# lenskit/lkpy

Hardware: AMD Instinct MI355X
Metric: ALS-implicit epochs/sec (ML-25M-shaped, k=64) (higher is better)
Workload: dtype f32; 1 GPU; MovieLens-25M-shaped, als-implicit k=64, 829 timed epochs, 1 x MI355X; solver=cholesky, n_items=62423, nnz=25000095, parallelism=single GPU

## Files before the change

### include/lkamd.h

```cpp
#ifndef LKAMD_H
#define LKAMD_H

#include <stddef.h>
#include <stdint.h>

#ifdef __cplusplus
extern "C" {
#endif

#define LK_OK 0
#define LK_E_INVALID (-1)
#define LK_E_HIP (-2)
#define LK_E_NOT_SPD (-3)
#define LK_E_NAN_SIM (-4)
#define LK_E_NOMEM (-5)
#define LK_E_CANCELLED (-6)

#define LK_SOLVER_CHOLESKY 0
#define LK_SOLVER_CG 1
#define LK_SOLVER_AUTO 2

const char *lk_last_error(void);
const char *lk_version(void);
int lk_device_count(void);
// ... 7 lines not shown

typedef struct lk_task_ctl lk_task_ctl;
int lk_task_ctl_create(lk_task_ctl **out);
void lk_task_ctl_destroy(lk_task_ctl *ctl);
void lk_task_ctl_cancel(lk_task_ctl *ctl);
int lk_task_ctl_cancelled(const lk_task_ctl *ctl);
void lk_task_ctl_reset(lk_task_ctl *ctl);
int lk_task_ctl_progress(const lk_task_ctl *ctl, int64_t *rows_done, int64_t *rows_total);

size_t lk_gramian_workspace_bytes(int32_t k);
int lk_gramian(const float *d_m, int64_t n, int32_t k, int32_t ld, float reg, float *d_out,
               int32_t ld_out, void *d_ws, void *stream);

typedef struct lk_als_plan lk_als_plan;

int lk_als_plan_create(lk_als_plan **out, const void *h_indptr, int indptr_is_64, int64_t n_rows,
                       int32_t k, int32_t solver);
#define LK_ALS_PLAN_REFERENCE_ORDER 1
#define LK_ALS_PLAN_HYBRID_ORDER 2
int lk_als_plan_create_ex(lk_als_plan **out, const void *h_indptr, int indptr_is_64,
                          int64_t n_rows, int32_t k, int32_t solver, int32_t flags);
void lk_als_plan_destroy(lk_als_plan *plan);
int64_t lk_als_plan_long_rows(const lk_als_plan *plan);
const float *lk_als_plan_yref(const lk_als_plan *plan, const void *d_ws);
size_t lk_als_plan_workspace_bytes(const lk_als_plan *plan);
int32_t lk_als_plan_solver(const lk_als_plan *plan);

int lk_als_plan_set_cg(lk_als_plan *plan, float tol, int32_t max_iter);
int lk_als_plan_cg_stats(const lk_als_plan *plan, void *d_ws, void *stream,
                         int64_t *out_iterations, int64_t *out_rows);
int lk_als_plan_set_ctl(lk_als_plan *plan, lk_task_ctl *ctl);
int64_t lk_als_plan_short_rows(const lk_als_plan *plan);
int64_t lk_als_plan_woodbury_rows(const lk_als_plan *plan);
int lk_als_plan_set_z(lk_als_plan *plan, const float *d_z);
int lk_als_plan_set_z_workspace(lk_als_plan *plan, float *d_zbuf);
int lk_als_plan_set_rhs_workspace(lk_als_plan *plan, float *d_y);
int lk_als_plan_set_z_shared(lk_als_plan *plan, const float *d_z, const void *d_flag);
int lk_als_plan_set_z_leader(lk_als_plan *plan, int on);
const void *lk_als_plan_z_flag(const lk_als_plan *plan, const void *d_ws);
size_t lk_spd_inverse_workspace_bytes(int32_t k);
int lk_spd_inverse(const float *d_a, int32_t lda, int32_t k, float *d_out, int32_t *d_flag,
                   void *d_ws, void *stream);

int lk_als_implicit_half_epoch(const lk_als_plan *plan, const void *d_indptr,
                               const int32_t *d_indices, const float *d_values, int64_t n_rows,
                               int64_t n_cols, int32_t k, float *d_this, int32_t ld_this,
// ... 410 lines not shown
```

### lkpy_amd/_native.py

```python

from __future__ import annotations

import ctypes
import os
import re
from ctypes import POINTER, c_char_p, c_float, c_int, c_int32, c_int64, c_size_t, c_void_p
from pathlib import Path

_PKG = Path(__file__).resolve().parent
LIB_PATH = Path(os.environ.get("LK_AMD_LIBRARY", _PKG / "_lkamd.so"))
HEADER_PATH = _PKG.parent / "include" / "lkamd.h"

LK_OK = 0
LK_E_INVALID = -1
LK_E_HIP = -2
LK_E_NOT_SPD = -3
LK_E_NAN_SIM = -4
LK_E_NOMEM = -5
LK_E_CANCELLED = -6

SOLVER_CHOLESKY = 0
SOLVER_CG = 1
SOLVER_AUTO = 2

# ... 49 lines not shown
        "lk_task_ctl_create": (c_int, [POINTER(vp)]),
        "lk_task_ctl_destroy": (None, [vp]),
        "lk_task_ctl_cancel": (None, [vp]),
        "lk_task_ctl_cancelled": (c_int, [vp]),
        "lk_task_ctl_reset": (None, [vp]),
        "lk_task_ctl_progress": (c_int, [vp, POINTER(c_int64), POINTER(c_int64)]),
        "lk_als_plan_set_ctl": (c_int, [vp, vp]),
        "lk_iknn_plan_set_ctl": (c_int, [vp, vp]),
        "lk_iknn_plan_enable_timing": (c_int, [vp, c_int]),
        "lk_iknn_plan_get_timing": (c_int, [vp, POINTER(ctypes.c_double), POINTER(c_int32)]),
        "lk_argtopn_workspace_bytes": (c_size_t, [c_int64, c_int64, c_int32]),
        "lk_gramian_workspace_bytes": (c_size_t, [c_int32]),
        "lk_gramian": (c_int, [vp, c_int64, c_int32, c_int32, c_float, vp, c_int32, vp, vp]),
        "lk_als_plan_create": (c_int, [POINTER(vp), vp, c_int, c_int64, c_int32, c_int32]),
        "lk_als_plan_create_ex": (c_int, [POINTER(vp), vp, c_int, c_int64, c_int32, c_int32,
                                          c_int32]),
        "lk_als_plan_destroy": (None, [vp]),
        "lk_als_plan_workspace_bytes": (c_size_t, [vp]),
        "lk_als_plan_solver": (c_int32, [vp]),
        "lk_als_plan_set_cg": (c_int, [vp, c_float, c_int32]),
        "lk_als_plan_cg_stats": (c_int, [vp, vp, vp, POINTER(c_int64), POINTER(c_int64)]),
        "lk_als_plan_short_rows": (c_int64, [vp]),
        "lk_als_plan_long_rows": (c_int64, [vp]),
        "lk_als_plan_yref": (vp, [vp, vp]),
        "lk_als_plan_woodbury_rows": (c_int64, [vp]),
        "lk_als_plan_set_z": (c_int, [vp, vp]),
        "lk_als_plan_set_z_workspace": (c_int, [vp, vp]),
        "lk_als_plan_set_rhs_workspace": (c_int, [vp, vp]),
        "lk_als_plan_set_z_shared": (c_int, [vp, vp, vp]),
        "lk_als_plan_set_z_leader": (c_int, [vp, c_int]),
        "lk_als_plan_z_flag": (vp, [vp, vp]),
        "lk_spd_inverse_workspace_bytes": (c_size_t, [c_int32]),
        "lk_spd_inverse": (c_int, [vp, c_int32, c_int32, vp, vp, vp, vp]),
        "lk_als_implicit_half_epoch": (
            c_int,
            [vp, vp, vp, vp, c_int64, c_int64, c_int32, vp, c_int32, vp, c_int32, vp, c_int32, vp,
             vp, vp],
        ),
        "lk_als_implicit_epoch": (
            c_int,
            [vp, vp, vp, vp, vp, vp, vp, vp, c_int32, vp, vp, vp, c_int32, c_float, vp, c_int32,
             c_float, vp, vp, vp, vp, vp],
        ),
        "lk_als_explicit_half_epoch": (
            c_int,
            [vp, vp, vp, vp, c_int64, c_int64, c_int32, vp, c_int32, vp, c_int32, c_float, vp, vp,
# ... 307 lines not shown
```

### lkpy_amd/csrc/als_chol.hip

```cpp
#include <algorithm>
#include <utility>

#include "als_plan.h"
#include "common.h"
#include "delta_reduce.h"

#ifndef LK_ALS_RING
#define LK_ALS_RING 4
#endif

namespace lk {

#ifdef LK_ALS_PHASES
__device__ unsigned *lk_als_phase_buf;
#define LK_PHASE_T(var) const unsigned long long var = __builtin_amdgcn_s_memtime()
#define LK_PHASE_ADD(i, a, b) \
    if (lane_id() == 0 && lk_als_phase_buf) lk_als_phase_buf[t * 8 + (i)] = (unsigned)((b) - (a))
#else
#define LK_PHASE_T(var)
#define LK_PHASE_ADD(i, a, b)
#endif

__host__ __device__ constexpr int als_tiles(int NT) { return NT * (NT + 1) / 2; }
__host__ __device__ constexpr int tidx(int ti, int tj) { return tj * (tj + 1) / 2 + ti; }
// ... 48 lines not shown
        q[3] = t.w;
    }
}

template <int NT>
struct GatherRing {
    static constexpr int RING = LK_ALS_RING;
    float q[RING][NT];
    float v[RING];
};

template <int NT>
__device__ __forceinline__ void ring_issue(GatherRing<NT> &R, const int slot_idx, const int g,
                                           const float *stage_slot,
                                           const float *__restrict__ other)
{
    constexpr int KP = NT * 16;
    const int lane = lane_id();
    const int col = __builtin_bit_cast(int, stage_slot[g * 4]);
    R.v[slot_idx] = stage_slot[64 + g * 4];
    load_q<NT>(other + (int64_t)col * KP + (lane & 15) * NT, R.q[slot_idx]);
}

template <int NT, bool MASKED, bool SEQY = false>
__device__ __forceinline__ void ring_consume(Gram<NT> &G, const GatherRing<NT> &R,
                                             const int slot_idx, const int g, const int nb,
                                             const bool expl)
{
    const int lane = lane_id();
    const bool live = !MASKED || (g * 4 + (lane >> 4)) < nb;
    const float v = R.v[slot_idx];
    const float va = expl ? 1.0f : v;
    float q[NT], a[NT];
#pragma unroll
    for (int t = 0; t < NT; ++t) {
        q[t] = live ? R.q[slot_idx][t] : 0.f;
        a[t] = q[t] * va;
    }
#pragma unroll
    for (int tj = 0; tj < NT; ++tj)
#pragma unroll
        for (int ti = 0; ti <= tj; ++ti)
            G.t[tidx(ti, tj)] = __builtin_amdgcn_mfma_f32_16x16x4f32(a[ti], q[tj],
                                                                     G.t[tidx(ti, tj)], 0, 0, 0);
    const float v1 = expl ? v : v + 1.0f;
    if constexpr (SEQY) {
        y_chain_step<NT>(G.yc, q, v1);
    } else {
#pragma unroll
        for (int t = 0; t < NT; ++t) G.y[t] = fmaf(q[t], v1, G.y[t]);
    }
}

constexpr int GRAM_STAGE_WORDS = 256;

template <int NT, bool SEQY = false>
__device__ __forceinline__ void gram_accumulate(Gram<NT> &G, const int32_t *__restrict__ cols,
                                                const float *__restrict__ vals, int64_t beg,
                                                int64_t end, const float *__restrict__ other,
                                                int , const bool expl,
                                                float *stage )
{
    const int lane = lane_id();
    constexpr int RING = GatherRing<NT>::RING;
    static_assert(RING >= 1 && RING <= 8 && 16 % RING == 0, "gather ring: 1, 2, 4 or 8 slots");
    GatherRing<NT> R;
    const int64_t last = end - 1;

    float *wr_cur = stage + lane, *wr_nxt = stage + 128 + lane;
    const float *rd_cur = stage + (lane >> 4), *rd_nxt = stage + 128 + (lane >> 4);
    int nxt_col;
    float nxt_val;
    {
        const int64_t e = (beg + lane < end) ? beg + lane : last;
        wr_cur[0] = __builtin_bit_cast(float, cols[e]);
        wr_cur[64] = vals[e];
    }
#pragma unroll
    for (int g = 0; g < RING; ++g) ring_issue<NT>(R, g, g, rd_cur, other);

    int64_t base = beg;
    for (; base + 64 <= end; base += 64) {
        {
            const int64_t e = (base + 64 + lane < end) ? base + 64 + lane : last;
            nxt_col = cols[e];
            nxt_val = vals[e];
        }
#pragma unroll
        for (int g = 0; g < 16; ++g) {
            ring_consume<NT, false, SEQY>(G, R, g % RING, g, 64, expl);
            if (g == 16 - RING - 2) {
                wr_nxt[0] = __builtin_bit_cast(float, nxt_col);
                wr_nxt[64] = nxt_val;
            }
            if (g < 16 - RING)
                ring_issue<NT>(R, g % RING, g + RING, rd_cur, other);
            else
                ring_issue<NT>(R, g % RING, g + RING - 16, rd_nxt, other);
            __builtin_amdgcn_sched_barrier(0);
        }
        float *tw = wr_cur;
        wr_cur = wr_nxt;
        wr_nxt = tw;
        const float *tr = rd_cur;
        rd_cur = rd_nxt;
        rd_nxt = tr;
    }
    if (base < end) {
        const int nb = (int)(end - base);
        const int ngroups = (nb + 3) >> 2;
#pragma unroll
        for (int g = 0; g < 16; ++g) {
            if (g < ngroups) ring_consume<NT, true, SEQY>(G, R, g % RING, g, nb, expl);
            if (g < 16 - RING) ring_issue<NT>(R, g % RING, g + RING, rd_cur, other);
        }
    }
}

#ifndef LK_ALS_DMA_RING
#define LK_ALS_DMA_RING 8
#endif
constexpr int DMA_RING = LK_ALS_DMA_RING;
constexpr int GRAM_DMA_WORDS = DMA_RING * 256;

template <int N>
__device__ __forceinline__ void wait_vm()
{
    asm volatile("s_waitcnt vmcnt(%0)" ::"n"(N) : "memory");
}
__device__ __forceinline__ void wait_vm_upto(const int n)
{
    if (n >= 7) wait_vm<7>();
    else if (n == 6) wait_vm<6>();
    else if (n == 5) wait_vm<5>();
    else if (n == 4) wait_vm<4>();
    else if (n == 3) wait_vm<3>();
    else if (n == 2) wait_vm<2>();
    else if (n == 1) wait_vm<1>();
    else wait_vm<0>();
}

__device__ __forceinline__ void dma_issue(const unsigned ring_lds, const int slot_idx, const int g,
                                          const float *stage_slot,
                                          const float *__restrict__ other)
{
    const int lane = lane_id();
// ... 3 lines not shown
    const unsigned dst = ring_lds + slot_idx * 1024;
    unsigned keep;
    asm volatile(
        "s_mov_b32 %0, m0\n\ts_mov_b32 m0, %2\n\ts_nop 0\n\t"
        "global_load_lds_dwordx4 %1, off\n\ts_mov_b32 m0, %0"
        : "=&s"(keep)
        : "v"(src), "s"(dst)
        : "memory");
}

struct DmaOperand {
    f32x4 q;
    float v;
};
__device__ __forceinline__ DmaOperand dma_fetch(const float *ring, const int slot_idx, const int g,
                                                const float *stage_slot)
{
    DmaOperand o;
    o.q = *reinterpret_cast<const f32x4 *>(ring + slot_idx * 256 + lane_id() * 4);
    o.v = stage_slot[64 + g * 4];
    return o;
}

template <bool MASKED, bool SEQY = false>
__device__ __forceinline__ void dma_apply(Gram<4> &G, const DmaOperand &o, const int g,
                                          const int nb, const bool expl)
{
    const int lane = lane_id();
    const bool live = !MASKED || (g * 4 + (lane >> 4)) < nb;
    const float v = o.v;
    const float va = expl ? 1.0f : v;
    float q[4] = {o.q.x, o.q.y, o.q.z, o.q.w}, a[4];
#pragma unroll
    for (int t = 0; t < 4; ++t) {
        q[t] = live ? q[t] : 0.f;
        a[t] = q[t] * va;
    }
#pragma unroll
    for (int tj = 0; tj < 4; ++tj)
#pragma unroll
        for (int ti = 0; ti <= tj; ++ti)
            G.t[tidx(ti, tj)] = __builtin_amdgcn_mfma_f32_16x16x4f32(a[ti], q[tj],
                                                                     G.t[tidx(ti, tj)], 0, 0, 0);
    const float v1 = expl ? v : v + 1.0f;
    if constexpr (SEQY) {
        y_chain_step<4>(G.yc, q, v1);
    } else {
#pragma unroll
        for (int t = 0; t < 4; ++t) G.y[t] = fmaf(q[t], v1, G.y[t]);
    }
}

template <bool MASKED, bool SEQY = false>
__device__ __forceinline__ void dma_consume(Gram<4> &G, const float *ring, const int slot_idx,
                                            const int g, const int nb, const float *stage_slot,
                                            const bool expl)
{
    dma_apply<MASKED, SEQY>(G, dma_fetch(ring, slot_idx, g, stage_slot), g, nb, expl);
}

template <int NT>
__host__ __device__ constexpr int slab_floats();
template <int NT>
__device__ __forceinline__ void slab_store(const Gram<NT> &G, float *__restrict__ slab);
template <int NT>
__device__ __forceinline__ void gram_zero(Gram<NT> &G);

template <bool SEQY = false>
__device__ __forceinline__ void gram_accumulate_dma(Gram<4> &G, const int32_t *__restrict__ cols,
                                                    const float *__restrict__ vals, int64_t beg,
                                                    int64_t end, const float *__restrict__ other,
                                                    const bool expl, float *ring, float *stage,
                                                    float *__restrict__ slab = nullptr)
{
    constexpr int RING = DMA_RING;
    static_assert(RING == 8 || RING == 4, "DMA ring: 4 or 8 groups");
    const int lane = lane_id();
    const int64_t last = end - 1;
    const unsigned ring_lds =
        __builtin_amdgcn_readfirstlane((unsigned)(uintptr_t) reinterpret_cast<void *>(ring));

    float *wr_cur = stage + lane, *wr_nxt = stage + 128 + lane;
    const float *rd_cur = stage + (lane >> 4), *rd_nxt = stage + 128 + (lane >> 4);
    {
        const int64_t e = (beg + lane < end) ? beg + lane : last;
        wr_cur[0] = __builtin_bit_cast(float, cols[e]);
        wr_cur[64] = vals[e];
    }
    const int total = (int)((end - beg + 3) >> 2);
#pragma unroll
    for (int g = 0; g < RING; ++g)
        if (g < total) dma_issue(ring_lds, g, g, rd_cur, other);

    int64_t base = beg;
    int g0 = 0;
    for (; g0 + 16 + RING <= total; base += 64, g0 += 16) {
        int nxt_col;
        float nxt_val;
        {
            const int64_t e = (base + 64 + lane < end) ? base + 64 + lane : last;
            nxt_col = cols[e];
            nxt_val = vals[e];
        }
        wait_vm<RING - 1>();
        DmaOperand cur = dma_fetch(ring, 0, 0, rd_cur);
#pragma unroll
        for (int g = 0; g < 16; ++g) {
            DmaOperand nxt = cur;
            if (g + 1 < 16) {
                wait_vm<RING - 2>();
                nxt = dma_fetch(ring, (g + 1) % RING, g + 1, rd_cur);
            }
            dma_apply<false, SEQY>(G, cur, g, 64, expl);
            if (g == 16 - RING - 2) {
                wr_nxt[0] = __builtin_bit_cast(float, nxt_col);
                wr_nxt[64] = nxt_val;
            }
            if (g < 16 - RING)
                dma_issue(ring_lds, g % RING, g + RING, rd_cur, other);
            else
                dma_issue(ring_lds, g % RING, g + RING - 16, rd_nxt, other);
            cur = nxt;
            __builtin_amdgcn_sched_barrier(0);
        }
        if (slab && ((g0 + 16) & 63) == 0) {
            slab_store<4>(G, slab);
            slab += slab_floats<4>();
            gram_zero<4>(G);
        }
        float *tw = wr_cur;
        wr_cur = wr_nxt;
        wr_nxt = tw;
        const float *tr = rd_cur;
        rd_cur = rd_nxt;
        rd_nxt = tr;
    }
    for (; g0 < total; base += 64, g0 += 16) {
        const int nb = (int)((end - base < 64) ? end - base : 64);
        const bool more = g0 + 16 < total;
        int nxt_col = 0;
        float nxt_val = 0.f;
        if (more) {
            const int64_t e = (base + 64 + lane < end) ? base + 64 + lane : last;
            nxt_col = cols[e];
            nxt_val = vals[e];
        }
#pragma unroll
        for (int g = 0; g < 16; ++g) {
            const int gg = g0 + g;
            if (gg < total) {
                const int later = total - 1 - gg;
                wait_vm_upto(later < RING - 1 ? later : RING - 1);
                dma_consume<true, SEQY>(G, ring, g % RING, g, nb, rd_cur, expl);
            }
            if (g == 16 - RING - 2 && more) {
                wr_nxt[0] = __builtin_bit_cast(float, nxt_col);
                wr_nxt[64] = nxt_val;
            }
            if (gg + RING < total) {
                if (g < 16 - RING)
                    dma_issue(ring_lds, g % RING, g + RING, rd_cur, other);
                else
                    dma_issue(ring_lds, g % RING, g + RING - 16, rd_nxt, other);
            }
        }
        if (slab && ((g0 + 16) & 63) == 0 && g0 + 16 < total) {
            slab_store<4>(G, slab);
            slab += slab_floats<4>();
            gram_zero<4>(G);
        }
        float *tw = wr_cur;
        wr_cur = wr_nxt;
        wr_nxt = tw;
        const float *tr = rd_cur;
        rd_cur = rd_nxt;
        rd_nxt = tr;
    }
}

__device__ __forceinline__ void gram_accumulate_dma_256(Gram<4> &G, const int32_t *__restrict__ cols,
                                                        const float *__restrict__ vals, int64_t beg,
                                                        const float *__restrict__ other,
                                                        const bool expl, float *ring, float *stage)
{
    constexpr int RING = DMA_RING, TOTAL = 64;
    const int lane = lane_id();
    const unsigned ring_lds =
        __builtin_amdgcn_readfirstlane((unsigned)(uintptr_t) reinterpret_cast<void *>(ring));
    float *const wr0 = stage + lane, *const wr1 = stage + 128 + lane;
    const float *const rd0 = stage + (lane >> 4), *const rd1 = stage + 128 + (lane >> 4);
    wr0[0] = __builtin_bit_cast(float, cols[beg + lane]);
    wr0[64] = vals[beg + lane];
#pragma unroll
    for (int g = 0; g < RING; ++g) dma_issue(ring_lds, g, g, rd0, other);
#pragma unroll
    for (int b = 0; b < 4; ++b) {
        float *const wr_nxt = (b & 1) ? wr0 : wr1;
        const float *const rd_cur = (b & 1) ? rd1 : rd0, *const rd_nxt = (b & 1) ? rd0 : rd1;
        int nxt_col = 0;
        float nxt_val = 0.f;
        if (b < 3) {
            nxt_col = cols[beg + 64 * (b + 1) + lane];
            nxt_val = vals[beg + 64 * (b + 1) + lane];
        }
        {
            const int later = TOTAL - 1 - 16 * b;
            wait_vm_upto(later < RING - 1 ? later : RING - 1);
        }
        DmaOperand cur = dma_fetch(ring, 0, 0, rd_cur);
#pragma unroll
        for (int g = 0; g < 16; ++g) {
            const int gg = 16 * b + g;
            DmaOperand nxt = cur;
            if (g + 1 < 16) {
                const int later = TOTAL - 1 - (gg + 1);
                const int issued_after = (gg + RING < TOTAL ? gg + RING - 1 : TOTAL - 1) - (gg + 1);
                wait_vm_upto(issued_after < later ? issued_after : later);
                nxt = dma_fetch(ring, (g + 1) % RING, g + 1, rd_cur);
            }
            dma_apply<false>(G, cur, g, 64, expl);
            if (g == 16 - RING - 2 && b < 3) {
                wr_nxt[0] = __builtin_bit_cast(float, nxt_col);
                wr_nxt[64] = nxt_val;
            }
            if (gg + RING < TOTAL) {
                if (g < 16 - RING)
                    dma_issue(ring_lds, g % RING, g + RING, rd_cur, other);
                else
                    dma_issue(ring_lds, g % RING, g + RING - 16, rd_nxt, other);
            }
            cur = nxt;
            __builtin_amdgcn_sched_barrier(0);
        }
    }
}

template <int NT>
__host__ __device__ constexpr int slab_floats()
{
    return (als_tiles(NT) * 4 + NT) * 64;
}

template <int NT>
__device__ __forceinline__ void slab_store(const Gram<NT> &G, float *__restrict__ slab)
{
    const int lane = lane_id();
#pragma unroll
    for (int e = 0; e < als_tiles(NT); ++e)
        __builtin_nontemporal_store(G.t[e], reinterpret_cast<f32x4 *>(slab + (e * 64 + lane) * 4));
#pragma unroll
    for (int t = 0; t < NT; ++t) slab[als_tiles(NT) * 256 + lane * NT + t] = G.y[t];
}

template <int NT>
__device__ __forceinline__ void slab_add(Gram<NT> &G, const float *__restrict__ slab)
{
    const int lane = lane_id();
#pragma unroll
    for (int e = 0; e < als_tiles(NT); ++e)
        G.t[e] += *reinterpret_cast<const f32x4 *>(slab + (e * 64 + lane) * 4);
#pragma unroll
    for (int t = 0; t < NT; ++t) G.y[t] += slab[als_tiles(NT) * 256 + lane * NT + t];
}

template <int NT>
__device__ __forceinline__ void gram_zero(Gram<NT> &G)
{
#pragma unroll
    for (int e = 0; e < als_tiles(NT); ++e) G.t[e] = f32x4{0.f, 0.f, 0.f, 0.f};
#pragma unroll
    for (int t = 0; t < NT; ++t) G.y[t] = 0.f;
}

__global__ __launch_bounds__(256) void slab_group_reduce_kernel(float *__restrict__ slabs,
                                                                int64_t slab_floats,
                                                                const int32_t *__restrict__ grp_head,
                                                                const int32_t *__restrict__ grp_cnt,
                                                                int parts)
{
    const int g = blockIdx.x / parts;
    const int64_t e = ((int64_t)(blockIdx.x - g * parts) * 256 + threadIdx.x) * 4;
    if (e >= slab_floats) return;
    float *head = slabs + (size_t)grp_head[g] * slab_floats + e;
    const int cnt = grp_cnt[g];
    f32x4 acc = *reinterpret_cast<const f32x4 *>(head);
    int c = 1;
    for (; c + 8 <= cnt; c += 8) {
        f32x4 v[8];
#pragma unroll
        for (int u = 0; u < 8; ++u)
            v[u] = __builtin_nontemporal_load(
                reinterpret_cast<const f32x4 *>(head + (size_t)(c + u) * slab_floats));
#pragma unroll
        for (int u = 0; u < 8; ++u) acc += v[u];
    }
    for (; c < cnt; ++c)
        acc += *reinterpret_cast<const f32x4 *>(head + (size_t)c * slab_floats);
    *reinterpret_cast<f32x4 *>(head) = acc;
}

int launch_slab_group_reduce(const lk_als_plan *p, float *slabs, size_t slab_floats, hipStream_t st)
{
    if (p->n_groups <= 0) return LK_OK;
    const int parts = (int)((slab_floats / 4 + 255) / 256);
    hipLaunchKernelGGL(slab_group_reduce_kernel, dim3((unsigned)(p->n_groups * parts)), dim3(256),
                       0, st, slabs, (int64_t)slab_floats, p->d_grp_head, p->d_grp_cnt, parts);
    LK_HIP_CHECK(hipGetLastError());
    return LK_OK;
}

template <int NT>
__host__ __device__ constexpr int chunk_lds_floats()
{
    return GRAM_STAGE_WORDS + (NT == 4 ? GRAM_DMA_WORDS : 0);
}

template <int NT, bool EXPL>
__device__ __forceinline__ void als_chunk_body(
    const int32_t *__restrict__ indices, const float *__restrict__ values,
    const int64_t *__restrict__ chunk_beg, const int32_t *__restrict__ chunk_len,
    int64_t n_chunks, const float *__restrict__ other, int ld, float *__restrict__ slabs,
    const int64_t blk, float *__restrict__ lds_flat,
    const int32_t *__restrict__ chunk_slab = nullptr, const int block_len = 0)
{
    constexpr bool DMA = NT == 4;
    float(*stage_all)[chunk_lds_floats<NT>()] =
        reinterpret_cast<float(*)[chunk_lds_floats<NT>()]>(lds_flat);
    const int wave = __builtin_amdgcn_readfirstlane(threadIdx.x >> 6);
    const int64_t c = blk * 4 + wave;
    if (c >= n_chunks) return;
    Gram<NT> G;
    gram_zero<NT>(G);
    const int64_t beg = chunk_beg[c];
    float *slab = slabs + (size_t)(chunk_slab ? chunk_slab[c] : c) * slab_floats<NT>();
    if constexpr (DMA) {
        const int len = chunk_len[c];
        if (block_len == 256 && len > 256) {
            gram_accumulate_dma(G, indices, values, beg, beg + len, other, EXPL,
                                stage_all[wave] + GRAM_STAGE_WORDS, stage_all[wave], slab);
            slab += (size_t)((len - 1) >> 8) * slab_floats<NT>();
        } else if (len == 256)
            gram_accumulate_dma_256(G, indices, values, beg, other, EXPL,
                                    stage_all[wave] + GRAM_STAGE_WORDS, stage_all[wave]);
        else
            gram_accumulate_dma(G, indices, values, beg, beg + len, other, EXPL,
                                stage_all[wave] + GRAM_STAGE_WORDS, stage_all[wave]);
    } else
        gram_accumulate<NT>(G, indices, values, beg, beg + chunk_len[c], other, ld, EXPL,
                            stage_all[wave]);
    slab_store<NT>(G, slab);
}

template <int NT, bool EXPL>
__global__ __launch_bounds__(256) void als_chunk_kernel(
    const int32_t *__restrict__ indices, const float *__restrict__ values,
    const int64_t *__restrict__ chunk_beg, const int32_t *__restrict__ chunk_len,
    int64_t n_chunks, const float *__restrict__ other, int ld, float *__restrict__ slabs,
    const int32_t *__restrict__ chunk_slab, int block_len)
{
    __shared__ __attribute__((aligned(16))) float lds_flat[4 * chunk_lds_floats<NT>()];
    als_chunk_body<NT, EXPL>(indices, values, chunk_beg, chunk_len, n_chunks, other, ld, slabs,
                             (int64_t)blockIdx.x, lds_flat, chunk_slab, block_len);
}

template <int KP>
struct LPack {
    __host__ __device__ static constexpr int c0(int j) { return (j + 1) & ~3; }
    __host__ __device__ static constexpr int off(int j)
    {
        const int m = j >> 2, r = j & 3;
        return 4 * KP * m - 8 * m * m + 4 * m + r * (KP - 4 * m);
    }
    static constexpr int SIZE = KP * KP / 2 + KP;
};

template <int NT>
__host__ __device__ constexpr int hybrid_lds_floats()
{
    return LPack<NT * 16>::SIZE + NT * 16 + 256;
}

template <int NT, int M>
__device__ __forceinline__ void hybrid_step(Gram<NT> &G, float &b, float &minpiv,
                                            float *__restrict__ lds, const int lane)
{
// ... 139 lines not shown
        return;
    }

    LK_PHASE_T(ph1);
    Gram<NT> G;
#pragma unroll
    for (int tj = 0; tj < NT; ++tj)
#pragma unroll
        for (int ti = 0; ti <= tj; ++ti)
#pragma unroll
            for (int r = 0; r < 4; ++r)
                G.t[tidx(ti, tj)][r] = otor_p[(ti * 16 + slot * 4 + r) * KP + tj * 16 + sub];
#pragma unroll
    for (int tt = 0; tt < NT; ++tt) G.y[tt] = 0.f;

    const int first_slab = row_slab[row];
    if (first_slab >= 0) {
        const int64_t n = end - beg;
        const bool refo = YREF && chunk_rt > 0;
        const int ch = refo ? chunk_rt : LK_ALS_CHUNK;
        const int ns = (int)((n + ch - 1) / ch);
        const int step = refo ? ns : (ns > LK_ALS_SLAB_GROUP ? LK_ALS_SLAB_GROUP : 1);
        for (int s = 0; s < ns; s += step)
            slab_add<NT>(G, slabs + (size_t)(first_slab + s) * slab_floats<NT>());
    } else {
        if constexpr (NT == 4)
            gram_accumulate_dma<SEQY && !YREF>(G, indices, values, beg, end, other, EXPL, lds,
                                               lds + LPack<KP>::SIZE + KP);
        else
            gram_accumulate<NT, SEQY && !YREF>(G, indices, values, beg, end, other, ld_other,
                                               EXPL, lds);
    }
    if (EXPL) {
        const float dg = reg * (float)(end - beg);
#pragma unroll
        for (int ti = 0; ti < NT; ++ti)
#pragma unroll
            for (int r = 0; r < 4; ++r)
                if (slot * 4 + r == sub && (slot * 4 + r) * NT + ti < k) G.t[tidx(ti, ti)][r] += dg;
    }

#ifdef LK_ALS_PHASES
    asm volatile("" : "+v"(G.t[0]), "+v"(G.t[als_tiles(NT) - 1]));
#endif
    LK_PHASE_T(ph2);
    if (SEQY && !YREF && first_slab < 0) {
#pragma unroll
// ... 353 lines not shown
                       otor, ld_otor, h.k, h.otor_p());
    LK_HIP_CHECK(hipGetLastError());
    return LK_OK;
}

template <int NT, bool IS64, bool EXPL>
static int chol_front(CholHalf &h, CholKind<NT, IS64, EXPL>)
{
    const lk_als_plan *p = h.p;
    hipStream_t st = h.st;
    float *slabs = h.slabs();
    h.tm = p->timing && p->timing_n < lk_als_plan::TIMING_RING;
    if (h.tm) LK_HIP_CHECK(hipEventRecord(p->ev[p->timing_n][0], st));
    h.n_solve = p->dense_limit >= 0 && p->dense_limit < h.n_rows ? p->dense_limit : h.n_rows;
    h.yref = p->hybrid ? reinterpret_cast<float *>(h.ws + p->off_yref)
                       : (p->ctl ? nullptr : p->d_yref);
    h.n_y = !h.yref ? 0 : (p->hybrid ? std::min<int64_t>(p->n_long, h.n_solve) : h.n_solve);
    h.sr = st;
    if (h.n_y > 0) {
        int rc = plan_fork_rhs(p, st, &h.sr);
        if (rc != LK_OK) return rc;
        h.forked = h.sr != st;
    }
    if (p->n_chunks > 0) {
        hipLaunchKernelGGL((als_chunk_kernel<NT, EXPL>),
                           dim3((unsigned)((p->n_chunks + 3) / 4)), dim3(256), 0, st,
                           h.indices, h.values, p->d_chunk_beg, p->d_chunk_len, p->n_chunks,
                           h.other, h.ld_other, slabs, p->d_chunk_slab,
                           p->unit > p->chunk ? (int)p->chunk : 0);
    }
    if (h.n_y > 0) {
        int rc = launch_rhs_reference(p, h.indptr, IS64 ? 1 : 0, h.indices, h.values, p->d_order,
                                      h.n_y, h.other, EXPL, h.yref, h.sr);
        if (rc != LK_OK) return rc;
    }
    if (p->n_chunks > 0) {
        hipStream_t sg = st;
        if (h.forked) {
            int rc = plan_rhs_wait_main(p, st);
            if (rc != LK_OK) return rc;
            sg = h.sr;
        }
        int rc = launch_slab_group_reduce(p, slabs, slab_floats<NT>(), sg);
        if (rc != LK_OK) return rc;
    }
    if (h.tm) LK_HIP_CHECK(hipEventRecord(p->ev[p->timing_n][1], st));
    LK_HIP_CHECK(hipGetLastError());
    return LK_OK;
}

template <int NT, bool IS64, bool EXPL>
static int chol_solve(CholHalf &h, CholKind<NT, IS64, EXPL>, hipEvent_t otor_ready)
{
    const lk_als_plan *p = h.p;
    hipStream_t st = h.st;
    using IT = typename IndPtr<IS64>::type;
    const IT *ip = static_cast<const IT *>(h.indptr);
    const int ref_chunk = (p->ref_order || p->hybrid) ? p->chunk : 0;
    const int64_t n_y = h.n_y, n_solve = h.n_solve;
    float *yref = h.yref;
    if (otor_ready) LK_HIP_CHECK(hipStreamWaitEvent(st, otor_ready, 0));
#define LK_SOLVE_LAUNCH(CTLV, YREFV, T0, NTASKS, YPTR, STREAM)                                \
    LK_SOLVE_LAUNCH_S(CTLV, YREFV, false, T0, NTASKS, YPTR, STREAM)
#define LK_SOLVE_LAUNCH_S(CTLV, YREFV, SEQV, T0, NTASKS, YPTR, STREAM)                        \
    hipLaunchKernelGGL((als_solve_kernel<NT, IS64, EXPL, CTLV, YREFV, SEQV>),                  \
                       dim3((unsigned)(((NTASKS) + 3) / 4)), dim3(256), 0, (STREAM), ip,       \
// ... 138 lines not shown
```

### lkpy_amd/csrc/als_plan.h

```cpp
#pragma once
#include <hip/hip_runtime.h>
#include <stdint.h>

#define LK_DELTA_BLOCKS 256

#ifndef LK_ALS_WB64_K128_DEFAULT
#define LK_ALS_WB64_K128_DEFAULT 64
#endif

#ifndef LK_ALS_CHUNK
#define LK_ALS_CHUNK 1024
#endif
#ifndef LK_ALS_LONG_ROW
#define LK_ALS_LONG_ROW 2048
#endif
#define LK_ALS_CHUNK_BLK LK_ALS_CHUNK
#ifndef LK_ALS_SLAB_GROUP
#define LK_ALS_SLAB_GROUP 16
#endif

struct lk_als_plan {
    int64_t n_rows = 0;
    int32_t k = 0, KP = 0, NT = 0, solver = 0;
    int32_t is64 = 0;
// ... 73 lines not shown
                float *ws, hipStream_t st);
int als_wb_launch(const lk_als_plan *p, const void *indptr, int is64, const int32_t *indices,
                  const float *values, int64_t t0, int64_t n_rows, float *this_,
                  const float *other, const float *z, float *row_delta, int *status,
                  hipStream_t st);
int als_wb4_launch(const lk_als_plan *p, const void *indptr, int is64, const int32_t *indices,
                   const float *values, int64_t t0, int64_t n_rows, float *this_,
                   const float *other, const float *z, float *row_delta, int *status,
                   hipStream_t st, int slots = 4);
int als_wb64_launch(const lk_als_plan *p, const void *indptr, int is64, const int32_t *indices,
                    const float *values, int64_t t0, int64_t t1, float *this_,
                    const float *other, const float *z, float *row_delta, int *status,
                    hipStream_t st);
size_t spd_inverse_workspace_bytes(int KP);
int spd_inverse(const float *a, int lda, int k, int KP, float *out, int *flag, void *ws,
                hipStream_t st);
int launch_rhs_reference(const lk_als_plan *p, const void *indptr, int is64,
                         const int32_t *indices, const float *values, const int32_t *order,
                         int64_t n_tasks, const float *other, bool expl, float *y_out,
                         hipStream_t st);
int plan_fork_rhs(const lk_als_plan *p, hipStream_t st, hipStream_t *side);
int plan_join_rhs(const lk_als_plan *p, hipStream_t st);
int plan_rhs_wait_main(const lk_als_plan *p, hipStream_t st);
int launch_slab_group_reduce(const lk_als_plan *p, float *slabs, size_t slab_floats, hipStream_t st);
int launch_delta_reduce(const float *row_delta, int64_t n_rows, float *partial, float *out_frob,
                        hipStream_t st);
int gramian_tail(const float *m, int64_t n, int k, int KP, float reg, float *out, int ld_out,
                 float *gram_ws, const float *row_delta, float *partial, float *out_delta,
                 float *next_otor_p, int *next_status, hipStream_t st);
int als_chol_epoch(const lk_als_plan *pu, const lk_als_plan *pi, const void *u_indptr,
                   const int32_t *u_indices, const float *u_values, const void *i_indptr,
                   const int32_t *i_indices, const float *i_values, float *P, float *Q,
                   float *qtq, int ld_qtq, float user_reg, float *ptp, int ld_ptp, float item_reg,
                   char *ws_u, char *ws_i, float *gram_ws, float *out_delta, hipStream_t st);
}
```

### lkpy_amd/csrc/als_plan.hip

```cpp
#include <stdlib.h>
#include <string.h>
#include <strings.h>

#include <algorithm>
#include <initializer_list>
#include <mutex>
#include <vector>

#include "als_plan.h"
#include "common.h"

namespace lk {

int plan_fork_rhs(const lk_als_plan *p, hipStream_t st, hipStream_t *side)
{
    *side = st;
    if (!p->side_streams) return LK_OK;
    if (!p->side_rhs) {
        p->side_rhs = lk::side_stream_acquire();
        LK_REQUIRE(p->side_rhs != nullptr, "als: no side stream");
        LK_HIP_CHECK(hipEventCreateWithFlags(&p->ev_fork_rhs, hipEventDisableTiming));
        LK_HIP_CHECK(hipEventCreateWithFlags(&p->ev_join_rhs, hipEventDisableTiming));
        LK_HIP_CHECK(hipEventCreateWithFlags(&p->ev_mid_rhs, hipEventDisableTiming));
        LK_HIP_CHECK(hipEventCreateWithFlags(&p->ev_tail_rhs, hipEventDisableTiming));
// ... 70 lines not shown
}
bool pack_pool_give(char *ptr, size_t cap)
{
    if (cap > PackPool::MAX_BYTES) return false;
    int dev = -1;
    if (hipGetDevice(&dev) != hipSuccess) return false;
    PackPool &pl = pack_pool();
    std::lock_guard<std::mutex> lock(pl.mu);
    for (int i = 0; i < PackPool::SLOTS; ++i)
        if (!pl.slot[i].ptr) {
            pl.slot[i].ptr = ptr;
            pl.slot[i].cap = cap;
            pl.slot[i].dev = dev;
            return true;
        }
    return false;
}
}

static bool switch_on(const char *name)
{
    const char *e = getenv(name);
    return !(e && e[0] == '0');
}

extern "C" int lk_als_plan_create_ex(lk_als_plan **out, const void *h_indptr, int indptr_is_64,
                                     int64_t n_rows, int32_t k, int32_t solver, int32_t flags);

extern "C" int lk_als_plan_create(lk_als_plan **out, const void *h_indptr, int indptr_is_64,
                                  int64_t n_rows, int32_t k, int32_t solver)
{
    const char *e = getenv("LK_ALS_RHS_ORDER");
    int32_t flags = LK_ALS_PLAN_HYBRID_ORDER;
    if (e && e[0]) {
        if (!strcasecmp(e, "accurate")) flags = 0;
        else if (!strcasecmp(e, "reference")) flags = LK_ALS_PLAN_REFERENCE_ORDER;
        else
            LK_REQUIRE(!strcasecmp(e, "auto") || !strcasecmp(e, "hybrid") || !strcasecmp(e, "default"),
                       "lk_als_plan_create: unknown LK_ALS_RHS_ORDER '%s' (auto / reference / accurate)",
                       e);
    }
    return lk_als_plan_create_ex(out, h_indptr, indptr_is_64, n_rows, k, solver, flags);
}

extern "C" int lk_als_plan_create_ex(lk_als_plan **out, const void *h_indptr, int indptr_is_64,
                                     int64_t n_rows, int32_t k, int32_t solver, int32_t flags)
// ... 100 lines not shown
    p->t_cg1 = first_at_most(cg_len / 4, t_cg, n_rows);

    p->t_wb4 = switch_on("LK_ALS_WB4") ? t_4 : n_rows;
    p->t_wb8 = switch_on("LK_ALS_WB8") ? t_8 : p->t_wb4;
    const char *e_k128 = getenv("LK_ALS_WB64_K128");
    const int k128 = e_k128 ? atoi(e_k128) : LK_ALS_WB64_K128_DEFAULT;
    const int64_t t_wb = (KP == 256 || k128 >= 64) ? t_64 : (k128 >= 32 ? t_32 : p->t_short);
    p->wb_rows = n_rows - t_wb;
    const bool wb64 = switch_on("LK_ALS_WB64");
    p->t_wb64 = wb64 ? t_wb : p->t_short;
    const bool wb128 = KP == 256 && wb64 && switch_on("LK_ALS_WB128") && t_128 < t_64;
    p->t_wb128 = wb128 ? t_128 : p->t_wb64;
    p->side_streams = switch_on("LK_ALS_SIDE_STREAM");
    p->chunk_dma = KP == 256 && switch_on("LK_BLK_CHUNK_DMA");

    std::vector<int32_t> row_slab((size_t)n_rows, -1);
    std::vector<int32_t> chunk_row, chunk_slab;
    std::vector<int64_t> chunk_beg;
    std::vector<int32_t> chunk_len;
    p->unit = p->chunk;
    if (p->hybrid && (KP == 64 || p->chunk_dma)) {
        const char *e = getenv("LK_ALS_REF_UNIT");
        int u = e ? atoi(e) : LK_ALS_CHUNK;
        if (u < p->chunk) u = p->chunk;
        p->unit = u / p->chunk * p->chunk;
    }
    const int64_t UNIT = p->unit;
    {
        for (int64_t r = 0; r < n_rows; ++r) {
            int64_t n = len(r);
            if (n > LONG_ROW) {
                row_slab[(size_t)r] = (int32_t)p->n_slabs;
                for (int64_t o = 0; o < n; o += UNIT) {
                    chunk_row.push_back((int32_t)r);
                    chunk_beg.push_back(start(r) + o);
                    chunk_len.push_back((int32_t)std::min<int64_t>(UNIT, n - o));
                    chunk_slab.push_back((int32_t)(p->n_slabs + o / CHUNK));
                }
                p->n_slabs += (n + CHUNK - 1) / CHUNK;
                p->n_long++;
            }
        }
    }
    if (p->n_slabs >= (int64_t)INT32_MAX) {
        delete p;
        lk::set_error("lk_als_plan_create: too many slabs");
// ... 158 lines not shown
        (void)hipDeviceSynchronize();
        if (!pack_pool_give(p->d_pack, p->pack_cap)) (void)hipFree(p->d_pack);
    }
    if (swap) (void)hipSetDevice(caller);
    delete p;
}

extern "C" size_t lk_als_plan_workspace_bytes(const lk_als_plan *p) { return p ? p->ws_bytes : 0; }
extern "C" int32_t lk_als_plan_solver(const lk_als_plan *p) { return p ? p->solver : -1; }

extern "C" int lk_als_plan_set_ctl(lk_als_plan *p, lk_task_ctl *ctl)
{
    LK_REQUIRE(p != nullptr, "lk_als_plan_set_ctl: null plan");
    p->ctl = ctl;
    return LK_OK;
}

extern "C" int64_t lk_als_plan_short_rows(const lk_als_plan *p)
{
    return p ? p->n_rows - p->t_short : 0;
}

extern "C" int64_t lk_als_plan_long_rows(const lk_als_plan *p) { return p ? p->n_long : 0; }

extern "C" const float *lk_als_plan_yref(const lk_als_plan *p, const void *d_ws)
{
    if (!p || !d_ws || !p->hybrid) return nullptr;
    return reinterpret_cast<const float *>(static_cast<const char *>(d_ws) + p->off_yref);
}

extern "C" int64_t lk_als_plan_woodbury_rows(const lk_als_plan *p) { return p ? p->wb_rows : 0; }

extern "C" int lk_als_plan_set_z(lk_als_plan *p, const float *d_z)
{
    LK_REQUIRE(p != nullptr, "lk_als_plan_set_z: null plan");
    p->d_z = d_z;
    return LK_OK;
}

extern "C" int lk_als_plan_set_z_shared(lk_als_plan *p, const float *d_z, const void *d_flag)
{
    LK_REQUIRE(p != nullptr, "lk_als_plan_set_z_shared: null plan");
    LK_REQUIRE((d_z == nullptr) == (d_flag == nullptr),
               "lk_als_plan_set_z_shared: Z and its flag word go together");
    LK_REQUIRE(d_z == nullptr || (p->KP > 64 && p->KP <= 256),
               "lk_als_plan_set_z_shared: the Woodbury kernels serve padded k = 128 / 256 only");
// ... 280 lines not shown
```

Baseline: 285.5 epochs/s.

## Skip RHS accumulation in chunk kernel when reference RHS covers long rows; adapt unit size

Adds a WITH_Y template switch so the long-row chunk Gram kernels skip accumulating and storing the RHS vector y when a separate reference-order RHS pass already covers all long rows. The slab group reduce then only sums the Gram tiles. The chunk DMA ring depth becomes its own knob, and the plan picks the reference unit size (1024/512/256) from the device CU count so there are enough work units to fill the GPU. This trims redundant FMAs and slab traffic and rebalances work granularity, at the cost of more template instantiations and a device query at plan creation.

```diff
diff --git a/include/lkamd.h b/include/lkamd.h
--- a/include/lkamd.h
+++ b/include/lkamd.h
@@ -53,6 +53,8 @@
                           int64_t n_rows, int32_t k, int32_t solver, int32_t flags);
 void lk_als_plan_destroy(lk_als_plan *plan);
 int64_t lk_als_plan_long_rows(const lk_als_plan *plan);
+int64_t lk_als_plan_units(const lk_als_plan *plan);
+int32_t lk_als_plan_unit(const lk_als_plan *plan);
 const float *lk_als_plan_yref(const lk_als_plan *plan, const void *d_ws);
 size_t lk_als_plan_workspace_bytes(const lk_als_plan *plan);
 int32_t lk_als_plan_solver(const lk_als_plan *plan);
diff --git a/lkpy_amd/_native.py b/lkpy_amd/_native.py
--- a/lkpy_amd/_native.py
+++ b/lkpy_amd/_native.py
@@ -95,6 +95,8 @@
         "lk_als_plan_cg_stats": (c_int, [vp, vp, vp, POINTER(c_int64), POINTER(c_int64)]),
         "lk_als_plan_short_rows": (c_int64, [vp]),
         "lk_als_plan_long_rows": (c_int64, [vp]),
+        "lk_als_plan_units": (c_int64, [vp]),
+        "lk_als_plan_unit": (c_int32, [vp]),
         "lk_als_plan_yref": (vp, [vp, vp]),
         "lk_als_plan_woodbury_rows": (c_int64, [vp]),
         "lk_als_plan_set_z": (c_int, [vp, vp]),
diff --git a/lkpy_amd/csrc/als_chol.hip b/lkpy_amd/csrc/als_chol.hip
--- a/lkpy_amd/csrc/als_chol.hip
+++ b/lkpy_amd/csrc/als_chol.hip
@@ -94,7 +94,7 @@
     load_q<NT>(other + (int64_t)col * KP + (lane & 15) * NT, R.q[slot_idx]);
 }
 
-template <int NT, bool MASKED, bool SEQY = false>
+template <int NT, bool MASKED, bool SEQY = false, bool WITH_Y = true>
 __device__ __forceinline__ void ring_consume(Gram<NT> &G, const GatherRing<NT> &R,
                                              const int slot_idx, const int g, const int nb,
                                              const bool expl)
@@ -115,18 +115,20 @@
         for (int ti = 0; ti <= tj; ++ti)
             G.t[tidx(ti, tj)] = __builtin_amdgcn_mfma_f32_16x16x4f32(a[ti], q[tj],
                                                                      G.t[tidx(ti, tj)], 0, 0, 0);
-    const float v1 = expl ? v : v + 1.0f;
-    if constexpr (SEQY) {
-        y_chain_step<NT>(G.yc, q, v1);
-    } else {
-#pragma unroll
-        for (int t = 0; t < NT; ++t) G.y[t] = fmaf(q[t], v1, G.y[t]);
+    if constexpr (WITH_Y) {
+        const float v1 = expl ? v : v + 1.0f;
+        if constexpr (SEQY) {
+            y_chain_step<NT>(G.yc, q, v1);
+        } else {
+#pragma unroll
+            for (int t = 0; t < NT; ++t) G.y[t] = fmaf(q[t], v1, G.y[t]);
+        }
     }
 }
 
 constexpr int GRAM_STAGE_WORDS = 256;
 
-template <int NT, bool SEQY = false>
+template <int NT, bool SEQY = false, bool WITH_Y = true>
 __device__ __forceinline__ void gram_accumulate(Gram<NT> &G, const int32_t *__restrict__ cols,
                                                 const float *__restrict__ vals, int64_t beg,
                                                 int64_t end, const float *__restrict__ other,
@@ -160,7 +162,7 @@
         }
 #pragma unroll
         for (int g = 0; g < 16; ++g) {
-            ring_consume<NT, false, SEQY>(G, R, g % RING, g, 64, expl);
+            ring_consume<NT, false, SEQY, WITH_Y>(G, R, g % RING, g, 64, expl);
             if (g == 16 - RING - 2) {
                 wr_nxt[0] = __builtin_bit_cast(float, nxt_col);
                 wr_nxt[64] = nxt_val;
@@ -183,7 +185,7 @@
         const int ngroups = (nb + 3) >> 2;
 #pragma unroll
         for (int g = 0; g < 16; ++g) {
-            if (g < ngroups) ring_consume<NT, true, SEQY>(G, R, g % RING, g, nb, expl);
+            if (g < ngroups) ring_consume<NT, true, SEQY, WITH_Y>(G, R, g % RING, g, nb, expl);
             if (g < 16 - RING) ring_issue<NT>(R, g % RING, g + RING, rd_cur, other);
         }
     }
@@ -193,7 +195,6 @@
 #define LK_ALS_DMA_RING 8
 #endif
 constexpr int DMA_RING = LK_ALS_DMA_RING;
-constexpr int GRAM_DMA_WORDS = DMA_RING * 256;
 
 template <int N>
 __device__ __forceinline__ void wait_vm()
@@ -243,7 +244,7 @@
     return o;
 }
 
-template <bool MASKED, bool SEQY = false>
+template <bool MASKED, bool SEQY = false, bool WITH_Y = true>
 __device__ __forceinline__ void dma_apply(Gram<4> &G, const DmaOperand &o, const int g,
                                           const int nb, const bool expl)
 {
@@ -263,38 +264,39 @@
         for (int ti = 0; ti <= tj; ++ti)
             G.t[tidx(ti, tj)] = __builtin_amdgcn_mfma_f32_16x16x4f32(a[ti], q[tj],
                                                                      G.t[tidx(ti, tj)], 0, 0, 0);
-    const float v1 = expl ? v : v + 1.0f;
-    if constexpr (SEQY) {
-        y_chain_step<4>(G.yc, q, v1);
-    } else {
-#pragma unroll
-        for (int t = 0; t < 4; ++t) G.y[t] = fmaf(q[t], v1, G.y[t]);
-    }
-}
-
-template <bool MASKED, bool SEQY = false>
+    if constexpr (WITH_Y) {
+        const float v1 = expl ? v : v + 1.0f;
+        if constexpr (SEQY) {
+            y_chain_step<4>(G.yc, q, v1);
+        } else {
+#pragma unroll
+            for (int t = 0; t < 4; ++t) G.y[t] = fmaf(q[t], v1, G.y[t]);
+        }
+    }
+}
+
+template <bool MASKED, bool SEQY = false, bool WITH_Y = true>
 __device__ __forceinline__ void dma_consume(Gram<4> &G, const float *ring, const int slot_idx,
                                             const int g, const int nb, const float *stage_slot,
                                             const bool expl)
 {
-    dma_apply<MASKED, SEQY>(G, dma_fetch(ring, slot_idx, g, stage_slot), g, nb, expl);
+    dma_apply<MASKED, SEQY, WITH_Y>(G, dma_fetch(ring, slot_idx, g, stage_slot), g, nb, expl);
 }
 
 template <int NT>
 __host__ __device__ constexpr int slab_floats();
-template <int NT>
+template <int NT, bool WITH_Y = true>
 __device__ __forceinline__ void slab_store(const Gram<NT> &G, float *__restrict__ slab);
-template <int NT>
+template <int NT, bool WITH_Y = true>
 __device__ __forceinline__ void gram_zero(Gram<NT> &G);
 
-template <bool SEQY = false>
+template <bool SEQY = false, bool WITH_Y = true, int RING = DMA_RING>
 __device__ __forceinline__ void gram_accumulate_dma(Gram<4> &G, const int32_t *__restrict__ cols,
                                                     const float *__restrict__ vals, int64_t beg,
                                                     int64_t end, const float *__restrict__ other,
                                                     const bool expl, float *ring, float *stage,
                                                     float *__restrict__ slab = nullptr)
 {
-    constexpr int RING = DMA_RING;
     static_assert(RING == 8 || RING == 4, "DMA ring: 4 or 8 groups");
     const int lane = lane_id();
     const int64_t last = end - 1;
@@ -332,7 +334,7 @@
                 wait_vm<RING - 2>();
                 nxt = dma_fetch(ring, (g + 1) % RING, g + 1, rd_cur);
             }
-            dma_apply<false, SEQY>(G, cur, g, 64, expl);
+            dma_apply<false, SEQY, WITH_Y>(G, cur, g, 64, expl);
             if (g == 16 - RING - 2) {
                 wr_nxt[0] = __builtin_bit_cast(float, nxt_col);
                 wr_nxt[64] = nxt_val;
@@ -345,9 +347,9 @@
             __builtin_amdgcn_sched_barrier(0);
         }
         if (slab && ((g0 + 16) & 63) == 0) {
-            slab_store<4>(G, slab);
+            slab_store<4, WITH_Y>(G, slab);
             slab += slab_floats<4>();
-            gram_zero<4>(G);
+            gram_zero<4, WITH_Y>(G);
         }
         float *tw = wr_cur;
         wr_cur = wr_nxt;
@@ -372,7 +374,7 @@
             if (gg < total) {
                 const int later = total - 1 - gg;
                 wait_vm_upto(later < RING - 1 ? later : RING - 1);
-                dma_consume<true, SEQY>(G, ring, g % RING, g, nb, rd_cur, expl);
+                dma_consume<true, SEQY, WITH_Y>(G, ring, g % RING, g, nb, rd_cur, expl);
             }
             if (g == 16 - RING - 2 && more) {
                 wr_nxt[0] = __builtin_bit_cast(float, nxt_col);
@@ -386,9 +388,9 @@
             }
         }
         if (slab && ((g0 + 16) & 63) == 0 && g0 + 16 < total) {
-            slab_store<4>(G, slab);
+            slab_store<4, WITH_Y>(G, slab);
             slab += slab_floats<4>();
-            gram_zero<4>(G);
+            gram_zero<4, WITH_Y>(G);
         }
         float *tw = wr_cur;
         wr_cur = wr_nxt;
@@ -399,12 +401,13 @@
     }
 }
 
+template <bool WITH_Y = true, int RING = DMA_RING>
 __device__ __forceinline__ void gram_accumulate_dma_256(Gram<4> &G, const int32_t *__restrict__ cols,
                                                         const float *__restrict__ vals, int64_t beg,
                                                         const float *__restrict__ other,
                                                         const bool expl, float *ring, float *stage)
 {
-    constexpr int RING = DMA_RING, TOTAL = 64;
+    constexpr int TOTAL = 64;
     const int lane = lane_id();
     const unsigned ring_lds =
         __builtin_amdgcn_readfirstlane((unsigned)(uintptr_t) reinterpret_cast<void *>(ring));
@@ -439,7 +442,7 @@
                 wait_vm_upto(issued_after < later ? issued_after : later);
                 nxt = dma_fetch(ring, (g + 1) % RING, g + 1, rd_cur);
             }
-            dma_apply<false>(G, cur, g, 64, expl);
+            dma_apply<false, false, WITH_Y>(G, cur, g, 64, expl);
             if (g == 16 - RING - 2 && b < 3) {
                 wr_nxt[0] = __builtin_bit_cast(float, nxt_col);
                 wr_nxt[64] = nxt_val;
@@ -462,46 +465,53 @@
     return (als_tiles(NT) * 4 + NT) * 64;
 }
 
-template <int NT>
+template <int NT, bool WITH_Y>
 __device__ __forceinline__ void slab_store(const Gram<NT> &G, float *__restrict__ slab)
 {
     const int lane = lane_id();
 #pragma unroll
     for (int e = 0; e < als_tiles(NT); ++e)
         __builtin_nontemporal_store(G.t[e], reinterpret_cast<f32x4 *>(slab + (e * 64 + lane) * 4));
-#pragma unroll
-    for (int t = 0; t < NT; ++t) slab[als_tiles(NT) * 256 + lane * NT + t] = G.y[t];
-}
-
-template <int NT>
+    if constexpr (WITH_Y) {
+#pragma unroll
+        for (int t = 0; t < NT; ++t) slab[als_tiles(NT) * 256 + lane * NT + t] = G.y[t];
+    }
+}
+
+template <int NT, bool WITH_Y = true>
 __device__ __forceinline__ void slab_add(Gram<NT> &G, const float *__restrict__ slab)
 {
     const int lane = lane_id();
 #pragma unroll
     for (int e = 0; e < als_tiles(NT); ++e)
         G.t[e] += *reinterpret_cast<const f32x4 *>(slab + (e * 64 + lane) * 4);
-#pragma unroll
-    for (int t = 0; t < NT; ++t) G.y[t] += slab[als_tiles(NT) * 256 + lane * NT + t];
-}
-
-template <int NT>
+    if constexpr (WITH_Y) {
+#pragma unroll
+        for (int t = 0; t < NT; ++t) G.y[t] += slab[als_tiles(NT) * 256 + lane * NT + t];
+    }
+}
+
+template <int NT, bool WITH_Y>
 __device__ __forceinline__ void gram_zero(Gram<NT> &G)
 {
 #pragma unroll
     for (int e = 0; e < als_tiles(NT); ++e) G.t[e] = f32x4{0.f, 0.f, 0.f, 0.f};
-#pragma unroll
-    for (int t = 0; t < NT; ++t) G.y[t] = 0.f;
+    if constexpr (WITH_Y) {
+#pragma unroll
+        for (int t = 0; t < NT; ++t) G.y[t] = 0.f;
+    }
 }
 
 __global__ __launch_bounds__(256) void slab_group_reduce_kernel(float *__restrict__ slabs,
                                                                 int64_t slab_floats,
+                                                                int64_t sum_floats,
                                                                 const int32_t *__restrict__ grp_head,
                                                                 const int32_t *__restrict__ grp_cnt,
                                                                 int parts)
 {
     const int g = blockIdx.x / parts;
     const int64_t e = ((int64_t)(blockIdx.x - g * parts) * 256 + threadIdx.x) * 4;
-    if (e >= slab_floats) return;
+    if (e >= sum_floats) return;
     float *head = slabs + (size_t)grp_head[g] * slab_floats + e;
     const int cnt = grp_cnt[g];
     f32x4 acc = *reinterpret_cast<const f32x4 *>(head);
@@ -520,23 +530,37 @@
     *reinterpret_cast<f32x4 *>(head) = acc;
 }
 
-int launch_slab_group_reduce(const lk_als_plan *p, float *slabs, size_t slab_floats, hipStream_t st)
+int launch_slab_group_reduce(const lk_als_plan *p, float *slabs, size_t slab_floats, hipStream_t st,
+                             size_t sum_floats)
 {
     if (p->n_groups <= 0) return LK_OK;
-    const int parts = (int)((slab_floats / 4 + 255) / 256);
+    if (sum_floats == 0) sum_floats = slab_floats;
+    const int parts = (int)((sum_floats / 4 + 255) / 256);
     hipLaunchKernelGGL(slab_group_reduce_kernel, dim3((unsigned)(p->n_groups * parts)), dim3(256),
-                       0, st, slabs, (int64_t)slab_floats, p->d_grp_head, p->d_grp_cnt, parts);
+                       0, st, slabs, (int64_t)slab_floats, (int64_t)sum_floats, p->d_grp_head,
+                       p->d_grp_cnt, parts);
     LK_HIP_CHECK(hipGetLastError());
     return LK_OK;
 }
 
+#ifndef LK_ALS_CHUNK_RING
+#define LK_ALS_CHUNK_RING 8
+#endif
+constexpr int CHUNK_RING = LK_ALS_CHUNK_RING;
+
 template <int NT>
 __host__ __device__ constexpr int chunk_lds_floats()
 {
-    return GRAM_STAGE_WORDS + (NT == 4 ? GRAM_DMA_WORDS : 0);
-}
-
-template <int NT, bool EXPL>
+    return GRAM_STAGE_WORDS + (NT == 4 ? CHUNK_RING * 256 : 0);
+}
+
+int als_chol_chunk_wgs_per_cu()
+{
+    const int by_lds = (int)(160 * 1024 / (4 * chunk_lds_floats<4>() * sizeof(float)));
+    return by_lds < 5 ? by_lds : 5;
+}
+
+template <int NT, bool EXPL, bool WITH_Y>
 __device__ __forceinline__ void als_chunk_body(
     const int32_t *__restrict__ indices, const float *__restrict__ values,
     const int64_t *__restrict__ chunk_beg, const int32_t *__restrict__ chunk_len,
@@ -551,28 +575,31 @@
     const int64_t c = blk * 4 + wave;
     if (c >= n_chunks) return;
     Gram<NT> G;
-    gram_zero<NT>(G);
+    gram_zero<NT, WITH_Y>(G);
     const int64_t beg = chunk_beg[c];
     float *slab = slabs + (size_t)(chunk_slab ? chunk_slab[c] : c) * slab_floats<NT>();
     if constexpr (DMA) {
         const int len = chunk_len[c];
         if (block_len == 256 && len > 256) {
-            gram_accumulate_dma(G, indices, values, beg, beg + len, other, EXPL,
-                                stage_all[wave] + GRAM_STAGE_WORDS, stage_all[wave], slab);
+            gram_accumulate_dma<false, WITH_Y, CHUNK_RING>(
+                G, indices, values, beg, beg + len, other, EXPL,
+                stage_all[wave] + GRAM_STAGE_WORDS, stage_all[wave], slab);
             slab += (size_t)((len - 1) >> 8) * slab_floats<NT>();
         } else if (len == 256)
-            gram_accumulate_dma_256(G, indices, values, beg, other, EXPL,
-                                    stage_all[wave] + GRAM_STAGE_WORDS, stage_all[wave]);
+            gram_accumulate_dma_256<WITH_Y, CHUNK_RING>(
+                G, indices, values, beg, other, EXPL, stage_all[wave] + GRAM_STAGE_WORDS,
+                stage_all[wave]);
         else
-            gram_accumulate_dma(G, indices, values, beg, beg + len, other, EXPL,
-                                stage_all[wave] + GRAM_STAGE_WORDS, stage_all[wave]);
+            gram_accumulate_dma<false, WITH_Y, CHUNK_RING>(
+                G, indices, values, beg, beg + len, other, EXPL,
+                stage_all[wave] + GRAM_STAGE_WORDS, stage_all[wave]);
     } else
-        gram_accumulate<NT>(G, indices, values, beg, beg + chunk_len[c], other, ld, EXPL,
-                            stage_all[wave]);
-    slab_store<NT>(G, slab);
-}
-
-template <int NT, bool EXPL>
+        gram_accumulate<NT, false, WITH_Y>(G, indices, values, beg, beg + chunk_len[c], other, ld,
+                                           EXPL, stage_all[wave]);
+    slab_store<NT, WITH_Y>(G, slab);
+}
+
+template <int NT, bool EXPL, bool WITH_Y>
 __global__ __launch_bounds__(256) void als_chunk_kernel(
     const int32_t *__restrict__ indices, const float *__restrict__ values,
     const int64_t *__restrict__ chunk_beg, const int32_t *__restrict__ chunk_len,
@@ -580,8 +607,8 @@
     const int32_t *__restrict__ chunk_slab, int block_len)
 {
     __shared__ __attribute__((aligned(16))) float lds_flat[4 * chunk_lds_floats<NT>()];
-    als_chunk_body<NT, EXPL>(indices, values, chunk_beg, chunk_len, n_chunks, other, ld, slabs,
-                             (int64_t)blockIdx.x, lds_flat, chunk_slab, block_len);
+    als_chunk_body<NT, EXPL, WITH_Y>(indices, values, chunk_beg, chunk_len, n_chunks, other, ld,
+                                     slabs, (int64_t)blockIdx.x, lds_flat, chunk_slab, block_len);
 }
 
 template <int KP>
@@ -767,7 +794,7 @@
         const int ns = (int)((n + ch - 1) / ch);
         const int step = refo ? ns : (ns > LK_ALS_SLAB_GROUP ? LK_ALS_SLAB_GROUP : 1);
         for (int s = 0; s < ns; s += step)
-            slab_add<NT>(G, slabs + (size_t)(first_slab + s) * slab_floats<NT>());
+            slab_add<NT, !YREF>(G, slabs + (size_t)(first_slab + s) * slab_floats<NT>());
     } else {
         if constexpr (NT == 4)
             gram_accumulate_dma<SEQY && !YREF>(G, indices, values, beg, end, other, EXPL, lds,
@@ -1167,12 +1194,18 @@
         if (rc != LK_OK) return rc;
         h.forked = h.sr != st;
     }
+    const bool chunk_y = !(h.yref != nullptr && h.n_y >= p->n_long);
     if (p->n_chunks > 0) {
-        hipLaunchKernelGGL((als_chunk_kernel<NT, EXPL>),
-                           dim3((unsigned)((p->n_chunks + 3) / 4)), dim3(256), 0, st,
-                           h.indices, h.values, p->d_chunk_beg, p->d_chunk_len, p->n_chunks,
-                           h.other, h.ld_other, slabs, p->d_chunk_slab,
-                           p->unit > p->chunk ? (int)p->chunk : 0);
+#define LK_CHUNK_LAUNCH(WITHY)                                                                  \
+    hipLaunchKernelGGL((als_chunk_kernel<NT, EXPL, WITHY>),                                    \
+                       dim3((unsigned)((p->n_chunks + 3) / 4)), dim3(256), 0, st, h.indices,   \
+                       h.values, p->d_chunk_beg, p->d_chunk_len, p->n_chunks, h.other,         \
+                       h.ld_other, slabs, p->d_chunk_slab, p->unit > p->chunk ? (int)p->chunk : 0)
+        if (chunk_y)
+            LK_CHUNK_LAUNCH(true);
+        else
+            LK_CHUNK_LAUNCH(false);
+#undef LK_CHUNK_LAUNCH
     }
     if (h.n_y > 0) {
         int rc = launch_rhs_reference(p, h.indptr, IS64 ? 1 : 0, h.indices, h.values, p->d_order,
@@ -1186,7 +1219,8 @@
             if (rc != LK_OK) return rc;
             sg = h.sr;
         }
-        int rc = launch_slab_group_reduce(p, slabs, slab_floats<NT>(), sg);
+        int rc = launch_slab_group_reduce(p, slabs, slab_floats<NT>(), sg,
+                                          chunk_y ? 0 : (size_t)als_tiles(NT) * 256);
         if (rc != LK_OK) return rc;
     }
     if (h.tm) LK_HIP_CHECK(hipEventRecord(p->ev[p->timing_n][1], st));
diff --git a/lkpy_amd/csrc/als_plan.h b/lkpy_amd/csrc/als_plan.h
--- a/lkpy_amd/csrc/als_plan.h
+++ b/lkpy_amd/csrc/als_plan.h
@@ -119,7 +119,9 @@
 int plan_fork_rhs(const lk_als_plan *p, hipStream_t st, hipStream_t *side);
 int plan_join_rhs(const lk_als_plan *p, hipStream_t st);
 int plan_rhs_wait_main(const lk_als_plan *p, hipStream_t st);
-int launch_slab_group_reduce(const lk_als_plan *p, float *slabs, size_t slab_floats, hipStream_t st);
+int launch_slab_group_reduce(const lk_als_plan *p, float *slabs, size_t slab_floats, hipStream_t st,
+                             size_t sum_floats = 0);
+int als_chol_chunk_wgs_per_cu();
 int launch_delta_reduce(const float *row_delta, int64_t n_rows, float *partial, float *out_frob,
                         hipStream_t st);
 int gramian_tail(const float *m, int64_t n, int k, int KP, float reg, float *out, int ld_out,
diff --git a/lkpy_amd/csrc/als_plan.hip b/lkpy_amd/csrc/als_plan.hip
--- a/lkpy_amd/csrc/als_plan.hip
+++ b/lkpy_amd/csrc/als_plan.hip
@@ -116,6 +116,21 @@
 {
     const char *e = getenv(name);
     return !(e && e[0] == '0');
+}
+
+static int device_cu_count(int dev)
+{
+    static std::mutex mu;
+    static int known[64] = {};
+    std::lock_guard<std::mutex> lock(mu);
+    const bool slot = dev >= 0 && dev < 64;
+    if (slot && known[dev] > 0) return known[dev];
+    int n = 0;
+    if (dev < 0 ||
+        hipDeviceGetAttribute(&n, hipDeviceAttributeMultiprocessorCount, dev) != hipSuccess || n < 0)
+        n = 0;
+    if (slot) known[dev] = n;
+    return n;
 }
 
 extern "C" int lk_als_plan_create_ex(lk_als_plan **out, const void *h_indptr, int indptr_is_64,
@@ -262,6 +277,24 @@
     if (p->hybrid && (KP == 64 || p->chunk_dma)) {
         const char *e = getenv("LK_ALS_REF_UNIT");
         int u = e ? atoi(e) : LK_ALS_CHUNK;
+        if (!e && KP == 64) {
+            const int cus = device_cu_count(p->device);
+            if (cus <= 0) {
+                delete p;
+                lk::set_error("lk_als_plan_create: cannot read the device's compute-unit count");
+                return LK_E_HIP;
+            }
+            const int64_t want = 2 * (int64_t)cus * lk::als_chol_chunk_wgs_per_cu() * 4;
+            int64_t units_1024 = 0, units_512 = 0;
+            for (int64_t r = 0; r < n_rows; ++r) {
+                const int64_t n = len(r);
+                if (n > LONG_ROW) {
+                    units_1024 += (n + 1023) / 1024;
+                    units_512 += (n + 511) / 512;
+                }
+            }
+            u = units_1024 >= want ? 1024 : (units_512 >= want ? 512 : 256);
+        }
         if (u < p->chunk) u = p->chunk;
         p->unit = u / p->chunk * p->chunk;
     }
@@ -466,6 +499,8 @@
 }
 
 extern "C" int64_t lk_als_plan_long_rows(const lk_als_plan *p) { return p ? p->n_long : 0; }
+extern "C" int64_t lk_als_plan_units(const lk_als_plan *p) { return p ? p->n_chunks : 0; }
+extern "C" int32_t lk_als_plan_unit(const lk_als_plan *p) { return p ? p->unit : 0; }
 
 extern "C" const float *lk_als_plan_yref(const lk_als_plan *p, const void *d_ws)
 {
```

Measured after the change: 291.0 epochs/s (median of 6 runs). +1.9%, better.
